# sanweiliti/RoHM

Hardware: NVIDIA H100
Metric: denoised motion clips/sec (145-frame, 1000-step PoseNet p_sample_loop) (higher is better)
Workload: dtype f32 (fp16 hi/lo error-compensated tensor-core GEMMs)

## Files before the change

### rohm_b200/csrc/attention.cu

```cuda
#include "attention.cuh"

#include <cmath>

#include "common.h"
#include "gemm.cuh"
#include "ptx.cuh"

namespace rohm {
namespace {

__device__ __forceinline__ float4 load_qkv4(const float* qkv, const float* qkv_lo, int f16, int64_t idx) {
  if (!f16) return *reinterpret_cast<const float4*>(qkv + idx);
  const uint2 h = *reinterpret_cast<const uint2*>(reinterpret_cast<const __half*>(qkv) + idx);
  const uint2 l = *reinterpret_cast<const uint2*>(reinterpret_cast<const __half*>(qkv_lo) + idx);
  const __half2 h0 = *reinterpret_cast<const __half2*>(&h.x), h1 = *reinterpret_cast<const __half2*>(&h.y);
  const __half2 l0 = *reinterpret_cast<const __half2*>(&l.x), l1 = *reinterpret_cast<const __half2*>(&l.y);
  return make_float4(__low2float(h0) + __low2float(l0), __high2float(h0) + __high2float(l0),
                     __low2float(h1) + __low2float(l1), __high2float(h1) + __high2float(l1));
}
template <int DH>
__global__ void __launch_bounds__(256) attention_kernel(const float* __restrict__ qkv, const float* __restrict__ qkv_lo,
                                                        float* __restrict__ ctx_hi, float* __restrict__ ctx_lo, int S,
                                                        int D, int H, float scale, int f16) {
  constexpr int KP = DH + 4;
// ... 359 lines not shown
  for (int i = threadIdx.x; i < 16 * NK * (DH / 8); i += blockDim.x) {
    const int s = i / (DH / 8), c = i % (DH / 8);
    const int sc = s < S ? s : S - 1;
    const uint32_t nbytes = s < S ? 16u : 0u;
    const __half* src = qkv_hi + (base + sc) * ld + h * DH + c * 8 + D;
    const uint32_t dst = ptx::smem_u32(Kh + s * P + c * 8);
    constexpr uint32_t plane = 16 * NK * P * 2;
    asm volatile("cp.async.cg.shared.global [%0], [%1], 16, %2;" ::"r"(dst), "l"(src), "r"(nbytes) : "memory");
    asm volatile("cp.async.cg.shared.global [%0], [%1], 16, %2;" ::"r"(dst + plane), "l"(src + lo_off), "r"(nbytes) : "memory");
    asm volatile("cp.async.cg.shared.global [%0], [%1], 16, %2;" ::"r"(dst + 2 * plane), "l"(src + D), "r"(nbytes) : "memory");
    asm volatile("cp.async.cg.shared.global [%0], [%1], 16, %2;" ::"r"(dst + 3 * plane), "l"(src + D + lo_off), "r"(nbytes)
                 : "memory");
  }
  asm volatile("cp.async.commit_group;" ::: "memory");

  const int r0 = warp * 16;
  const int rowA = min(r0 + g, S - 1), rowB = min(r0 + g + 8, S - 1);
  const __half* qA = qkv_hi + (base + rowA) * ld + h * DH + 2 * t;
  const int dB = (rowB - rowA) * ld;
  auto ldq = [](const __half* p) { return __ldg(reinterpret_cast<const unsigned int*>(p)); };
  uint32_t qh[4] = {ldq(qA), ldq(qA + dB), ldq(qA + 8), ldq(qA + dB + 8)};
  uint32_t ql[4] = {ldq(qA + lo_off), ldq(qA + lo_off + dB), ldq(qA + lo_off + 8), ldq(qA + lo_off + dB + 8)};
  asm volatile("cp.async.wait_group 0;" ::: "memory");
  __syncthreads();

  float acc[NT][4];
#pragma unroll
  for (int j = 0; j < NT; ++j) acc[j][0] = acc[j][1] = acc[j][2] = acc[j][3] = 0.0f;
  const int lm = lane >> 3, lr = lane & 7;
  const __half* kbase = (lm < 2 ? Kh : Kl) + lr * P + (lm & 1) * 8;
#pragma unroll 1
  for (int k = 0; k < DH / 16; ++k) {
    uint32_t ah[4], al[4];
#pragma unroll
    for (int i = 0; i < 4; ++i) ah[i] = qh[i], al[i] = ql[i];
    if (k + 1 < DH / 16) {
      const __half* q = qA + 16 * (k + 1);
      qh[0] = ldq(q), qh[1] = ldq(q + dB), qh[2] = ldq(q + 8), qh[3] = ldq(q + dB + 8);
      q += lo_off;
      ql[0] = ldq(q), ql[1] = ldq(q + dB), ql[2] = ldq(q + 8), ql[3] = ldq(q + dB + 8);
    }
    const __half* kp = kbase + 16 * k;
#pragma unroll
    for (int j0 = 0; j0 < NT; j0 += 4) {
      uint32_t bf[4][4];
#pragma unroll
      for (int u = 0; u < 4; ++u) ldmatrix_x4(bf[u], kp + (j0 + u) * 8 * P);
#pragma unroll
      for (int u = 0; u < 4; ++u) mma_f16_16x8x16(acc[j0 + u], al, bf[u][0], bf[u][1]);
#pragma unroll
      for (int u = 0; u < 4; ++u) mma_f16_16x8x16(acc[j0 + u], ah, bf[u][2], bf[u][3]);
#pragma unroll
      for (int u = 0; u < 4; ++u) mma_f16_16x8x16(acc[j0 + u], ah, bf[u][0], bf[u][1]);
    }
  }

  float mxA = -INFINITY, mxB = -INFINITY;
#pragma unroll
  for (int j = 0; j < NT; ++j) {
#pragma unroll
    for (int e = 0; e < 2; ++e) {
      const bool ok = (8 * j + 2 * t + e) < S;
      acc[j][e] = ok ? acc[j][e] * scale : -INFINITY;
      acc[j][2 + e] = ok ? acc[j][2 + e] * scale : -INFINITY;
      mxA = fmaxf(mxA, acc[j][e]);
      mxB = fmaxf(mxB, acc[j][2 + e]);
    }
  }
  mxA = fmaxf(mxA, __shfl_xor_sync(0xffffffffu, mxA, 1));
  mxA = fmaxf(mxA, __shfl_xor_sync(0xffffffffu, mxA, 2));
  mxB = fmaxf(mxB, __shfl_xor_sync(0xffffffffu, mxB, 1));
  mxB = fmaxf(mxB, __shfl_xor_sync(0xffffffffu, mxB, 2));
  float sumA = 0.0f, sumB = 0.0f;
#pragma unroll
  for (int j = 0; j < NT; ++j) {
#pragma unroll
    for (int e = 0; e < 2; ++e) {
      acc[j][e] = expf(acc[j][e] - mxA);
      acc[j][2 + e] = expf(acc[j][2 + e] - mxB);
      sumA += acc[j][e];
      sumB += acc[j][2 + e];
    }
  }
  sumA += __shfl_xor_sync(0xffffffffu, sumA, 1);
  sumA += __shfl_xor_sync(0xffffffffu, sumA, 2);
  sumB += __shfl_xor_sync(0xffffffffu, sumB, 1);
  sumB += __shfl_xor_sync(0xffffffffu, sumB, 2);
  const float invA = 1.0f / sumA, invB = 1.0f / sumB;

  uint32_t ph[NK][4], pl[NK][4];
#pragma unroll
  for (int jj = 0; jj < NK; ++jj) {
    split_f16x2(acc[2 * jj][0] * invA, acc[2 * jj][1] * invA, ph[jj][0], pl[jj][0]);
    split_f16x2(acc[2 * jj][2] * invB, acc[2 * jj][3] * invB, ph[jj][1], pl[jj][1]);
    split_f16x2(acc[2 * jj + 1][0] * invA, acc[2 * jj + 1][1] * invA, ph[jj][2], pl[jj][2]);
    split_f16x2(acc[2 * jj + 1][2] * invB, acc[2 * jj + 1][3] * invB, ph[jj][3], pl[jj][3]);
  }

  const bool okA = (r0 + g) < S, okB = (r0 + g + 8) < S;
  const int64_t oA = (base + r0 + g) * D + h * DH + 2 * t;
  const int64_t oB = oA + static_cast<int64_t>(8) * D;
  const __half* vbase = (lm < 2 ? Vh : Vl) + ((lm & 1) * 8 + lr) * P;
  constexpr int NU = 4;
#pragma unroll 1
  for (int n0 = 0; n0 < DH / 8; n0 += NU) {
    float o[NU][4];
#pragma unroll
    for (int u = 0; u < NU; ++u) o[u][0] = o[u][1] = o[u][2] = o[u][3] = 0.0f;
    const __half* vp = vbase + 8 * n0;
#pragma unroll
    for (int jj = 0; jj < NK; ++jj) {
      uint32_t bf[NU][4];
#pragma unroll
      for (int u = 0; u < NU; ++u) ldmatrix_x4_trans(bf[u], vp + 16 * jj * P + 8 * u);
#pragma unroll
      for (int u = 0; u < NU; ++u) mma_f16_16x8x16(o[u], pl[jj], bf[u][0], bf[u][1]);
#pragma unroll
      for (int u = 0; u < NU; ++u) mma_f16_16x8x16(o[u], ph[jj], bf[u][2], bf[u][3]);
#pragma unroll
      for (int u = 0; u < NU; ++u) mma_f16_16x8x16(o[u], ph[jj], bf[u][0], bf[u][1]);
    }
#pragma unroll
    for (int u = 0; u < NU; ++u) {
      const int n = n0 + u;
      uint32_t hA, lA, hB, lB;
      split_f16x2(o[u][0], o[u][1], hA, lA);
      split_f16x2(o[u][2], o[u][3], hB, lB);
      if (okA) {
        *reinterpret_cast<uint32_t*>(ctx_hi + oA + 8 * n) = hA;
        *reinterpret_cast<uint32_t*>(ctx_lo + oA + 8 * n) = lA;
      }
      if (okB) {
        *reinterpret_cast<uint32_t*>(ctx_hi + oB + 8 * n) = hB;
        *reinterpret_cast<uint32_t*>(ctx_lo + oB + 8 * n) = lB;
      }
    }
  }
}

template <int DH>
size_t attention_f16_smem_bytes(int NK) { return sizeof(__half) * 4 * 16 * NK * attn_f16_pitch<DH>(); }

struct AttnWgParams {
  CUtensorMap q_hi, q_lo;
  CUtensorMap kv_hi, kv_lo;
  __half* ctx_hi;
  __half* ctx_lo;
  int S, D, H;
  float scale;
  const int* clip_off;
  const int* clip_ids;
};
constexpr int kAwKeys = 160;
constexpr int kAwQRows = 64;
constexpr int kAwQBuf = kAwQRows * 128;
constexpr int kAwKBuf = kAwKeys * 128;
constexpr int kAwSmemBytes = 4 * kAwQBuf + 8 * kAwKBuf + 1024;

__global__ void __launch_bounds__(128, 1) attention_wgmma_kernel(const __grid_constant__ AttnWgParams p) {
  extern __shared__ uint8_t aw_smem_raw[];
  __shared__ uint64_t bar_qk, bar_v;
  const uint32_t raw = ptx::smem_u32(aw_smem_raw);
  uint8_t* const sm = aw_smem_raw + ((1024u - (raw & 1023u)) & 1023u);
  uint8_t* const Qb = sm;
  uint8_t* const Kb = sm + 4 * kAwQBuf;
  uint8_t* const Vb = Kb + 4 * kAwKBuf;
  const int qtiles = (p.S + kAwQRows - 1) / kAwQRows;
  const int qt = static_cast<int>(blockIdx.x) % qtiles;
  const int bh = static_cast<int>(blockIdx.x) / qtiles;
  const int h = bh % p.H, b = bh / p.H;
  const int q0 = qt * kAwQRows;
  int S = p.S, row0 = b * p.S;
  if (p.clip_off != nullptr) {
    const int c = p.clip_ids[b];
    row0 = p.clip_off[c];
    S = p.clip_off[c + 1] - row0;
    if (q0 >= S) return;
  }
  const int warp = threadIdx.x >> 5, lane = threadIdx.x & 31;
  if (threadIdx.x == 0) {
    ptx::prefetch_tmap(&p.q_hi);
    ptx::prefetch_tmap(&p.q_lo);
    ptx::prefetch_tmap(&p.kv_hi);
    ptx::prefetch_tmap(&p.kv_lo);
    ptx::mbar_init(&bar_qk, 1);
    ptx::mbar_init(&bar_v, 1);
    ptx::fence_barrier_init();
  }
  __syncthreads();
  ptx::pdl_launch_dependents();
  ptx::pdl_wait_prior_grid();
  if (threadIdx.x == 0) {
    ptx::mbar_expect_tx(&bar_qk, 4 * kAwQBuf + 4 * kAwKBuf);
    for (int pl = 0; pl < 2; ++pl)
      for (int c = 0; c < 2; ++c) {
        ptx::tma_load_2d(Qb + (pl * 2 + c) * kAwQBuf, pl ? &p.q_lo : &p.q_hi, &bar_qk, h * 128 + 64 * c, row0 + q0);
        ptx::tma_load_2d(Kb + (pl * 2 + c) * kAwKBuf, pl ? &p.kv_lo : &p.kv_hi, &bar_qk, p.D + h * 128 + 64 * c, row0);
      }
    ptx::mbar_expect_tx(&bar_v, 4 * kAwKBuf);
    for (int pl = 0; pl < 2; ++pl)
      for (int c = 0; c < 2; ++c)
        ptx::tma_load_2d(Vb + (pl * 2 + c) * kAwKBuf, pl ? &p.kv_lo : &p.kv_hi, &bar_v, 2 * p.D + h * 128 + 64 * c, row0);
  }

  float s[80];
#pragma unroll
  for (int i = 0; i < 80; ++i) s[i] = 0.0f;
  ptx::mbar_wait(&bar_qk, 0);
  ptx::wgmma_fence_regs(s);
  ptx::wgmma_fence();
#pragma unroll
  for (int k = 0; k < 8; ++k) {
    const int c = k >> 2;
    const uint64_t ko = static_cast<uint64_t>((k & 3) * 2);
    const uint64_t qh = ptx::make_desc_kmajor<128>(ptx::smem_u32(Qb + c * kAwQBuf)) + ko;
    const uint64_t ql = ptx::make_desc_kmajor<128>(ptx::smem_u32(Qb + (2 + c) * kAwQBuf)) + ko;
    const uint64_t kh = ptx::make_desc_kmajor<128>(ptx::smem_u32(Kb + c * kAwKBuf)) + ko;
    const uint64_t kl = ptx::make_desc_kmajor<128>(ptx::smem_u32(Kb + (2 + c) * kAwKBuf)) + ko;
    ptx::wgmma_f16(s, ql, kh);
    ptx::wgmma_f16(s, qh, kl);
    ptx::wgmma_f16(s, qh, kh);
  }
  ptx::wgmma_commit();
  ptx::wgmma_wait<0>();
  ptx::wgmma_fence_regs(s);

  const int c2 = 2 * (lane & 3);
  float m0 = -INFINITY, m1 = -INFINITY;
#pragma unroll
  for (int j = 0; j < 20; ++j) {
#pragma unroll
    for (int e = 0; e < 2; ++e) {
      const bool valid = 8 * j + c2 + e < S;
      s[4 * j + e] = valid ? s[4 * j + e] : -INFINITY;
      s[4 * j + 2 + e] = valid ? s[4 * j + 2 + e] : -INFINITY;
      m0 = fmaxf(m0, s[4 * j + e]);
      m1 = fmaxf(m1, s[4 * j + 2 + e]);
    }
  }
#pragma unroll
  for (int off = 1; off <= 2; off <<= 1) {
    m0 = fmaxf(m0, __shfl_xor_sync(0xffffffffu, m0, off));
    m1 = fmaxf(m1, __shfl_xor_sync(0xffffffffu, m1, off));
  }
  float l0 = 0.0f, l1 = 0.0f;
#pragma unroll
  for (int j = 0; j < 20; ++j) {
#pragma unroll
    for (int e = 0; e < 2; ++e) {
      const bool valid = 8 * j + c2 + e < S;
      const float p0 = valid ? expf((s[4 * j + e] - m0) * p.scale) : 0.0f;
      const float p1 = valid ? expf((s[4 * j + 2 + e] - m1) * p.scale) : 0.0f;
      s[4 * j + e] = p0, s[4 * j + 2 + e] = p1;
      l0 += p0, l1 += p1;
    }
  }
#pragma unroll
  for (int off = 1; off <= 2; off <<= 1) {
    l0 += __shfl_xor_sync(0xffffffffu, l0, off);
    l1 += __shfl_xor_sync(0xffffffffu, l1, off);
  }
  uint32_t ph[10][4], plo[10][4];
#pragma unroll
  for (int k = 0; k < 10; ++k)
#pragma unroll
    for (int i = 0; i < 4; ++i) ptx::split_f16x2(s[8 * k + 2 * i], s[8 * k + 2 * i + 1], ph[k][i], plo[k][i]);
#pragma unroll
  for (int k = 0; k < 10; ++k)
#pragma unroll
    for (int i = 0; i < 4; ++i) asm volatile("" : "+r"(ph[k][i]), "+r"(plo[k][i])::"memory");

  ptx::mbar_wait(&bar_v, 0);
  if (S < kAwKeys) {
    const int n = (kAwKeys - S) * 8;
    for (int i = threadIdx.x; i < 4 * n; i += 128) {
      const int buf = i / n, r = i - buf * n;
      *reinterpret_cast<uint4*>(Vb + buf * kAwKBuf + S * 128 + r * 16) = make_uint4(0u, 0u, 0u, 0u);
    }
    ptx::fence_proxy_async();
    __syncthreads();
  }

  float o[64];
#pragma unroll
  for (int i = 0; i < 64; ++i) o[i] = 0.0f;
  ptx::wgmma_fence_regs(o);
  ptx::wgmma_fence();
#pragma unroll
  for (int k = 0; k < 10; ++k) {
    const uint64_t vh = ptx::make_desc_mnmajor_sw128(ptx::smem_u32(Vb + k * 2048), kAwKBuf, 1024);
    const uint64_t vl = ptx::make_desc_mnmajor_sw128(ptx::smem_u32(Vb + 2 * kAwKBuf + k * 2048), kAwKBuf, 1024);
    ptx::wgmma_f16_rs_tb(o, plo[k], vh);
    ptx::wgmma_f16_rs_tb(o, ph[k], vl);
    ptx::wgmma_f16_rs_tb(o, ph[k], vh);
  }
  ptx::wgmma_commit();
  ptx::wgmma_wait<0>();
  ptx::wgmma_fence_regs(o);
#pragma unroll
  for (int k = 0; k < 10; ++k)
#pragma unroll
    for (int i = 0; i < 4; ++i) asm volatile("" : "+r"(ph[k][i]), "+r"(plo[k][i])::"memory");

  const int ra = q0 + warp * 16 + (lane >> 2), rb = ra + 8;
  const float ia = 1.0f / l0, ib = 1.0f / l1;
#pragma unroll
  for (int j = 0; j < 16; ++j) {
    const int col = h * 128 + 8 * j + c2;
    uint32_t hi, lo;
    if (ra < S) {
      ptx::split_f16x2(o[4 * j] * ia, o[4 * j + 1] * ia, hi, lo);
      const int64_t off = static_cast<int64_t>(row0 + ra) * p.D + col;
      *reinterpret_cast<uint32_t*>(p.ctx_hi + off) = hi;
      *reinterpret_cast<uint32_t*>(p.ctx_lo + off) = lo;
    }
    if (rb < S) {
      ptx::split_f16x2(o[4 * j + 2] * ib, o[4 * j + 3] * ib, hi, lo);
      const int64_t off = static_cast<int64_t>(row0 + rb) * p.D + col;
      *reinterpret_cast<uint32_t*>(p.ctx_hi + off) = hi;
      *reinterpret_cast<uint32_t*>(p.ctx_lo + off) = lo;
    }
  }
}

struct AttnStreamParams {
  CUtensorMap hi, lo;
  __half* ctx_hi;
  __half* ctx_lo;
  int S, D, H;
  float scale;
  const int* clip_off;
  const int* clip_ids;
};
constexpr int kAsBlock = 64;
constexpr int kAsBuf = kAsBlock * 128;
constexpr int kAsTile = 4 * kAsBuf;
constexpr int kAsStages = 2;
constexpr int kAsSmemBytes = (1 + 2 * kAsStages) * kAsTile + 1024;

__global__ void __launch_bounds__(128, 1) attention_wgmma_stream_kernel(const __grid_constant__ AttnStreamParams p) {
  extern __shared__ uint8_t as_smem_raw[];
  __shared__ uint64_t bar_q, bar_k[kAsStages], bar_v[kAsStages];
  const uint32_t raw = ptx::smem_u32(as_smem_raw);
  uint8_t* const sm = as_smem_raw + ((1024u - (raw & 1023u)) & 1023u);
  uint8_t* const Qb = sm;
  uint8_t* const Kb = sm + kAsTile;
  uint8_t* const Vb = Kb + kAsStages * kAsTile;
  const int qtiles = (p.S + kAsBlock - 1) / kAsBlock;
  const int qt = static_cast<int>(blockIdx.x) % qtiles;
  const int bh = static_cast<int>(blockIdx.x) / qtiles;
  const int h = bh % p.H, b = bh / p.H;
  const int q0 = qt * kAsBlock;
  int S = p.S, row0 = b * p.S;
  if (p.clip_off != nullptr) {
    const int c = p.clip_ids[b];
    row0 = p.clip_off[c];
    S = p.clip_off[c + 1] - row0;
    if (q0 >= S) return;
  }
  const int nblk = (S + kAsBlock - 1) / kAsBlock;
  const int kcol = p.D + h * 128, vcol = 2 * p.D + h * 128;
  const int warp = threadIdx.x >> 5, lane = threadIdx.x & 31;
  if (threadIdx.x == 0) {
    ptx::prefetch_tmap(&p.hi);
    ptx::prefetch_tmap(&p.lo);
    ptx::mbar_init(&bar_q, 1);
    for (int s = 0; s < kAsStages; ++s) ptx::mbar_init(&bar_k[s], 1), ptx::mbar_init(&bar_v[s], 1);
    ptx::fence_barrier_init();
  }
  __syncthreads();
  ptx::pdl_launch_dependents();
  ptx::pdl_wait_prior_grid();
  auto load_tile = [&](uint8_t* dst, uint64_t* bar, int col, int row) {
    ptx::mbar_expect_tx(bar, kAsTile);
    for (int pl = 0; pl < 2; ++pl)
      for (int c = 0; c < 2; ++c) ptx::tma_load_2d(dst + (pl * 2 + c) * kAsBuf, pl ? &p.lo : &p.hi, bar, col + 64 * c, row);
  };
  if (threadIdx.x == 0) {
    load_tile(Qb, &bar_q, h * 128, row0 + q0);
    for (int j = 0; j < kAsStages && j < nblk; ++j) {
      load_tile(Kb + j * kAsTile, &bar_k[j], kcol, row0 + j * kAsBlock);
      load_tile(Vb + j * kAsTile, &bar_v[j], vcol, row0 + j * kAsBlock);
    }
  }

  const int c2 = 2 * (lane & 3);
  float o[64];
#pragma unroll
  for (int i = 0; i < 64; ++i) o[i] = 0.0f;
  float m0 = -INFINITY, m1 = -INFINITY;
  float l0 = 0.0f, l1 = 0.0f;
  ptx::mbar_wait(&bar_q, 0);
#pragma unroll 1
  for (int j = 0; j < nblk; ++j) {
    const int st = j % kAsStages;
    const uint32_t phase = (j / kAsStages) & 1;
    uint8_t* const Ks = Kb + st * kAsTile;
    uint8_t* const Vs = Vb + st * kAsTile;
    const int kb = j * kAsBlock;

    float s[32];
#pragma unroll
    for (int i = 0; i < 32; ++i) s[i] = 0.0f;
    ptx::mbar_wait(&bar_k[st], phase);
    ptx::wgmma_fence_regs(s);
    ptx::wgmma_fence();
#pragma unroll
    for (int k = 0; k < 8; ++k) {
      const int c = k >> 2;
      const uint64_t ko = static_cast<uint64_t>((k & 3) * 2);
      const uint64_t qh = ptx::make_desc_kmajor<128>(ptx::smem_u32(Qb + c * kAsBuf)) + ko;
      const uint64_t ql = ptx::make_desc_kmajor<128>(ptx::smem_u32(Qb + (2 + c) * kAsBuf)) + ko;
      const uint64_t kh = ptx::make_desc_kmajor<128>(ptx::smem_u32(Ks + c * kAsBuf)) + ko;
      const uint64_t kl = ptx::make_desc_kmajor<128>(ptx::smem_u32(Ks + (2 + c) * kAsBuf)) + ko;
      ptx::wgmma_f16(s, ql, kh);
      ptx::wgmma_f16(s, qh, kl);
      ptx::wgmma_f16(s, qh, kh);
    }
    ptx::wgmma_commit();
    ptx::wgmma_wait<0>();
    ptx::wgmma_fence_regs(s);
    __syncthreads();
    if (threadIdx.x == 0 && j + kAsStages < nblk) load_tile(Ks, &bar_k[st], kcol, row0 + kb + kAsStages * kAsBlock);

    float n0 = m0, n1 = m1;
#pragma unroll
    for (int jj = 0; jj < 8; ++jj) {
#pragma unroll
      for (int e = 0; e < 2; ++e) {
        const bool valid = kb + 8 * jj + c2 + e < S;
        s[4 * jj + e] = valid ? s[4 * jj + e] : -INFINITY;
        s[4 * jj + 2 + e] = valid ? s[4 * jj + 2 + e] : -INFINITY;
        n0 = fmaxf(n0, s[4 * jj + e]);
        n1 = fmaxf(n1, s[4 * jj + 2 + e]);
      }
    }
#pragma unroll
    for (int off = 1; off <= 2; off <<= 1) {
      n0 = fmaxf(n0, __shfl_xor_sync(0xffffffffu, n0, off));
      n1 = fmaxf(n1, __shfl_xor_sync(0xffffffffu, n1, off));
    }
    const float a0 = expf((m0 - n0) * p.scale), a1 = expf((m1 - n1) * p.scale);
    m0 = n0, m1 = n1;
    float b0 = 0.0f, b1 = 0.0f;
#pragma unroll
    for (int jj = 0; jj < 8; ++jj) {
#pragma unroll
      for (int e = 0; e < 2; ++e) {
        const bool valid = kb + 8 * jj + c2 + e < S;
        const float p0 = valid ? expf((s[4 * jj + e] - m0) * p.scale) : 0.0f;
        const float p1 = valid ? expf((s[4 * jj + 2 + e] - m1) * p.scale) : 0.0f;
        s[4 * jj + e] = p0, s[4 * jj + 2 + e] = p1;
        b0 += p0, b1 += p1;
      }
    }
    l0 = l0 * a0 + b0, l1 = l1 * a1 + b1;
    uint32_t ph[4][4], plo[4][4];
#pragma unroll
    for (int k = 0; k < 4; ++k)
#pragma unroll
      for (int i = 0; i < 4; ++i) ptx::split_f16x2(s[8 * k + 2 * i], s[8 * k + 2 * i + 1], ph[k][i], plo[k][i]);

    ptx::mbar_wait(&bar_v[st], phase);
    if (kb + kAsBlock > S) {
      const int n = (kb + kAsBlock - S) * 8;
      for (int i = threadIdx.x; i < 4 * n; i += 128) {
        const int buf = i / n, r = i - buf * n;
        *reinterpret_cast<uint4*>(Vs + buf * kAsBuf + (S - kb) * 128 + r * 16) = make_uint4(0u, 0u, 0u, 0u);
      }
      ptx::fence_proxy_async();
      __syncthreads();
    }

    float ob[64];
#pragma unroll
    for (int i = 0; i < 64; ++i) ob[i] = 0.0f;
    ptx::wgmma_fence_regs(ob);
    ptx::wgmma_fence();
#pragma unroll
    for (int k = 0; k < 4; ++k) {
      const uint64_t vh = ptx::make_desc_mnmajor_sw128(ptx::smem_u32(Vs + k * 2048), kAsBuf, 1024);
      const uint64_t vl = ptx::make_desc_mnmajor_sw128(ptx::smem_u32(Vs + 2 * kAsBuf + k * 2048), kAsBuf, 1024);
      ptx::wgmma_f16_rs_tb(ob, plo[k], vh);
      ptx::wgmma_f16_rs_tb(ob, ph[k], vl);
      ptx::wgmma_f16_rs_tb(ob, ph[k], vh);
    }
    ptx::wgmma_commit();
    ptx::wgmma_wait<0>();
    ptx::wgmma_fence_regs(ob);
#pragma unroll
    for (int i = 0; i < 64; ++i) o[i] = fmaf(o[i], (i & 2) ? a1 : a0, ob[i]);
#pragma unroll
    for (int k = 0; k < 4; ++k)
#pragma unroll
      for (int i = 0; i < 4; ++i) asm volatile("" : "+r"(ph[k][i]), "+r"(plo[k][i])::"memory");
    __syncthreads();
    if (threadIdx.x == 0 && j + kAsStages < nblk) load_tile(Vs, &bar_v[st], vcol, row0 + kb + kAsStages * kAsBlock);
  }

#pragma unroll
  for (int off = 1; off <= 2; off <<= 1) {
    l0 += __shfl_xor_sync(0xffffffffu, l0, off);
    l1 += __shfl_xor_sync(0xffffffffu, l1, off);
  }
  const int ra = q0 + warp * 16 + (lane >> 2), rb = ra + 8;
  const float ia = 1.0f / l0, ib = 1.0f / l1;
#pragma unroll
  for (int j = 0; j < 16; ++j) {
    const int col = h * 128 + 8 * j + c2;
    uint32_t hi, lo;
    if (ra < S) {
      ptx::split_f16x2(o[4 * j] * ia, o[4 * j + 1] * ia, hi, lo);
      const int64_t off = static_cast<int64_t>(row0 + ra) * p.D + col;
      *reinterpret_cast<uint32_t*>(p.ctx_hi + off) = hi;
      *reinterpret_cast<uint32_t*>(p.ctx_lo + off) = lo;
    }
    if (rb < S) {
      ptx::split_f16x2(o[4 * j + 2] * ib, o[4 * j + 3] * ib, hi, lo);
      const int64_t off = static_cast<int64_t>(row0 + rb) * p.D + col;
      *reinterpret_cast<uint32_t*>(p.ctx_hi + off) = hi;
      *reinterpret_cast<uint32_t*>(p.ctx_lo + off) = lo;
    }
  }
}

size_t attention_mma_smem_bytes(int NT) { return sizeof(float) * 2 * 8 * NT * kAttnPitch; }

template <int DH, int NT>
cudaError_t launch_attention_mma(const AttnArgs& a, cudaStream_t st, bool pdl) {
  auto kern = attention_mma_kernel<DH, NT>;
  static bool attr_set = false;
  const size_t smem = attention_mma_smem_bytes(NT);
  if (!attr_set) {
    cudaError_t e = cudaFuncSetAttribute(kern, cudaFuncAttributeMaxDynamicSharedMemorySize, static_cast<int>(smem));
    if (e != cudaSuccess) return e;
    attr_set = true;
  }
  const int warps = (a.S + 15) / 16;
  return launch_chain(kern, dim3(a.B * a.H), dim3(32 * warps), smem, st, pdl, static_cast<const float*>(a.qkv_hi),
                      static_cast<float*>(a.ctx_hi), static_cast<float*>(a.ctx_lo), a.S, a.D, a.H, a.scale,
                      a.kind == kKindF16 ? 1 : 0);
}

template <int DH, int NK>
cudaError_t launch_attention_f16(const AttnArgs& a, cudaStream_t st, bool pdl) {
  const int warps = (a.S + 15) / 16;
  return launch_chain(attention_f16_kernel<DH, NK>, dim3(a.B * a.H), dim3(32 * warps), attention_f16_smem_bytes<DH>(NK), st,
                      pdl, static_cast<const __half*>(a.qkv_hi), static_cast<const __half*>(a.qkv_lo),
                      static_cast<__half*>(a.ctx_hi), static_cast<__half*>(a.ctx_lo), a.S, a.D, a.H, a.scale);
}

}

size_t attention_smem_bytes(int S, int DH) {
  const int Sp = (S + 31) & ~31;
  return sizeof(float) * (static_cast<size_t>(S) * (DH + 4) + static_cast<size_t>(S) * DH + 8 * DH + 8 * Sp);
}

int attention_wgmma_maps(AttnWgmmaMaps* maps, const AttnArgs& a) {
  const int D = a.D;
  int rc = make_tile_tmap_f16_sw128(&maps->q_hi, a.qkv_hi, a.rows, 3 * D, 3 * D, kAwQRows);
  if (rc == 0) rc = make_tile_tmap_f16_sw128(&maps->q_lo, a.qkv_lo, a.rows, 3 * D, 3 * D, kAwQRows);
  if (rc == 0) rc = make_tile_tmap_f16_sw128(&maps->kv_hi, a.qkv_hi, a.rows, 3 * D, 3 * D, kAwKeys);
  if (rc == 0) rc = make_tile_tmap_f16_sw128(&maps->kv_lo, a.qkv_lo, a.rows, 3 * D, 3 * D, kAwKeys);
  return rc;
}

cudaError_t attention_init_attributes(int max_tokens, int dh) {
  cudaError_t ea = cudaSuccess;
  auto set = [&](auto kern, size_t bytes) {
    if (ea == cudaSuccess) ea = cudaFuncSetAttribute(kern, cudaFuncAttributeMaxDynamicSharedMemorySize, static_cast<int>(bytes));
  };
  set(attention_mma_kernel<128, 4>, attention_mma_smem_bytes(4));
  set(attention_mma_kernel<128, 8>, attention_mma_smem_bytes(8));
  set(attention_mma_kernel<128, 12>, attention_mma_smem_bytes(12));
  set(attention_mma_kernel<128, 16>, attention_mma_smem_bytes(16));
  set(attention_mma_kernel<128, 20>, attention_mma_smem_bytes(20));
  set(attention_mma_kernel<64, 8>, attention_mma_smem_bytes(8));
  set(attention_mma_kernel<64, 20>, attention_mma_smem_bytes(20));
  set(attention_f16_kernel<128, 2>, attention_f16_smem_bytes<128>(2));
  set(attention_f16_kernel<128, 4>, attention_f16_smem_bytes<128>(4));
  set(attention_f16_kernel<128, 6>, attention_f16_smem_bytes<128>(6));
  set(attention_f16_kernel<128, 8>, attention_f16_smem_bytes<128>(8));
  set(attention_f16_kernel<128, 10>, attention_f16_smem_bytes<128>(10));
  set(attention_f16_kernel<64, 4>, attention_f16_smem_bytes<64>(4));
  set(attention_f16_kernel<64, 10>, attention_f16_smem_bytes<64>(10));
  set(attention_wgmma_kernel, kAwSmemBytes);
  set(attention_wgmma_stream_kernel, kAsSmemBytes);
  if (dh != 64 && dh != 128) return ea == cudaSuccess ? cudaErrorInvalidValue : ea;
  int simt_tokens = max_tokens < kAttnSimtMaxTokens ? max_tokens : kAttnSimtMaxTokens;
  while (simt_tokens > 1 && attention_smem_bytes(simt_tokens, dh) > kAttnSmemLimit) --simt_tokens;
  if (dh == 128) set(attention_kernel<128>, attention_smem_bytes(simt_tokens, 128));
  else set(attention_kernel<64>, attention_smem_bytes(simt_tokens, 64));
  return ea;
}

cudaError_t launch_attention(const AttnArgs& a, int which, const AttnWgmmaMaps* wg, cudaStream_t st, bool pdl) {
  const bool packed = a.clip_off != nullptr;
  if (a.B <= 0 || a.S <= 0 || a.H <= 0 || a.D % a.H != 0 || (packed ? a.S > a.rows : static_cast<int64_t>(a.B) * a.S > a.rows))
    return cudaErrorInvalidValue;
  if (packed && (a.clip_ids == nullptr || which == kAttnAuto)) return cudaErrorInvalidValue;
  const int dh = a.D / a.H;
  if (dh != 64 && dh != 128) return cudaErrorInvalidValue;
  const bool f16 = a.kind == kKindF16;
  const bool wg_ok = f16 && dh == 128 && a.S <= kAwKeys && wg != nullptr;
  const bool stream_ok = f16 && dh == 128 && wg != nullptr;
  const bool mma_ok = a.S <= kAttnWgmmaMaxTokens;
  if (which == kAttnAuto)
    which = wg_ok ? kAttnWgmma : (stream_ok && !mma_ok) ? kAttnWgmmaStream : !mma_ok ? kAttnSimt : f16 ? kAttnMmaF16 : kAttnMmaTf32;
  const int S = a.S;
  if (which == kAttnWgmmaStream) {
    if (!stream_ok) return cudaErrorInvalidValue;
    AttnStreamParams prm;
    prm.hi = wg->q_hi, prm.lo = wg->q_lo;
    prm.ctx_hi = static_cast<__half*>(a.ctx_hi), prm.ctx_lo = static_cast<__half*>(a.ctx_lo);
    prm.S = S, prm.D = a.D, prm.H = a.H, prm.scale = a.scale;
    prm.clip_off = a.clip_off, prm.clip_ids = a.clip_ids;
    const int qtiles = (S + kAsBlock - 1) / kAsBlock;
    return launch_chain(attention_wgmma_stream_kernel, dim3(a.B * a.H * qtiles), dim3(128), kAsSmemBytes, st, pdl, prm);
  }
  if (which == kAttnWgmma) {
    if (!wg_ok) return cudaErrorInvalidValue;
    AttnWgParams prm;
    prm.q_hi = wg->q_hi, prm.q_lo = wg->q_lo, prm.kv_hi = wg->kv_hi, prm.kv_lo = wg->kv_lo;
    prm.ctx_hi = static_cast<__half*>(a.ctx_hi), prm.ctx_lo = static_cast<__half*>(a.ctx_lo);
    prm.S = S, prm.D = a.D, prm.H = a.H, prm.scale = a.scale;
    prm.clip_off = a.clip_off, prm.clip_ids = a.clip_ids;
    const int qtiles = (S + kAwQRows - 1) / kAwQRows;
    return launch_chain(attention_wgmma_kernel, dim3(a.B * a.H * qtiles), dim3(128), kAwSmemBytes, st, pdl, prm);
  }
  if (packed) return cudaErrorInvalidValue;
  if (which == kAttnMmaF16) {
    if (!f16 || !mma_ok) return cudaErrorInvalidValue;
    const int nk = (S + 15) / 16;
    if (dh == 128 && nk <= 2) return launch_attention_f16<128, 2>(a, st, pdl);
    if (dh == 128 && nk <= 4) return launch_attention_f16<128, 4>(a, st, pdl);
    if (dh == 128 && nk <= 6) return launch_attention_f16<128, 6>(a, st, pdl);
    if (dh == 128 && nk <= 8) return launch_attention_f16<128, 8>(a, st, pdl);
    if (dh == 128) return launch_attention_f16<128, 10>(a, st, pdl);
    if (nk <= 4) return launch_attention_f16<64, 4>(a, st, pdl);
    return launch_attention_f16<64, 10>(a, st, pdl);
  }
  if (which == kAttnMmaTf32) {
    if (f16 || !mma_ok) return cudaErrorInvalidValue;
    const int nt = (S + 7) / 8;
    if (dh == 128 && nt <= 4) return launch_attention_mma<128, 4>(a, st, pdl);
    if (dh == 128 && nt <= 8) return launch_attention_mma<128, 8>(a, st, pdl);
    if (dh == 128 && nt <= 12) return launch_attention_mma<128, 12>(a, st, pdl);
    if (dh == 128 && nt <= 16) return launch_attention_mma<128, 16>(a, st, pdl);
    if (dh == 128) return launch_attention_mma<128, 20>(a, st, pdl);
    if (nt <= 8) return launch_attention_mma<64, 8>(a, st, pdl);
    return launch_attention_mma<64, 20>(a, st, pdl);
  }
  if (which == kAttnSimt) {
    const size_t smem = attention_smem_bytes(S, dh);
    if (S > kAttnSimtMaxTokens || smem > kAttnSmemLimit) return cudaErrorInvalidValue;
    auto kern = dh == 128 ? attention_kernel<128> : attention_kernel<64>;
    return launch_chain(kern, dim3(a.B * a.H), dim3(256), smem, st, pdl, static_cast<const float*>(a.qkv_hi),
                        static_cast<const float*>(a.qkv_lo), static_cast<float*>(a.ctx_hi), static_cast<float*>(a.ctx_lo), S,
                        a.D, a.H, a.scale, f16 ? 1 : 0);
  }
  return cudaErrorInvalidValue;
}

}
```

### rohm_b200/csrc/ptx.cuh

```cuda
#pragma once
#include <cstdint>
#include <cuda.h>
#include <cuda_fp16.h>
#include <cuda_runtime.h>

namespace rohm {
namespace ptx {

__device__ __forceinline__ uint32_t smem_u32(const void* p) {
  return static_cast<uint32_t>(__cvta_generic_to_shared(p));
}

__device__ __forceinline__ bool elect_one() {
  uint32_t pred = 0;
  asm volatile(
      "{\n\t"
      ".reg .pred P;\n\t"
      "elect.sync _|P, 0xffffffff;\n\t"
      "selp.u32 %0, 1, 0, P;\n\t"
      "}\n"
      : "=r"(pred));
  return pred != 0;
}

__device__ __forceinline__ void mbar_init(uint64_t* bar, uint32_t count) {
  asm volatile("mbarrier.init.shared::cta.b64 [%0], %1;" ::"r"(smem_u32(bar)), "r"(count));
}
__device__ __forceinline__ void fence_barrier_init() {
  asm volatile("fence.mbarrier_init.release.cluster;" ::: "memory");
}
__device__ __forceinline__ void fence_proxy_async() {
  asm volatile("fence.proxy.async.shared::cta;" ::: "memory");
}
__device__ __forceinline__ void mbar_expect_tx(uint64_t* bar, uint32_t bytes) {
  asm volatile("mbarrier.arrive.expect_tx.shared::cta.b64 _, [%0], %1;" ::"r"(smem_u32(bar)), "r"(bytes)
               : "memory");
}
__device__ __forceinline__ void mbar_arrive(uint64_t* bar) {
  asm volatile("mbarrier.arrive.shared::cta.b64 _, [%0];" ::"r"(smem_u32(bar)) : "memory");
}
__device__ __forceinline__ bool mbar_try_wait(uint64_t* bar, uint32_t parity) {
  uint32_t ok;
  asm volatile(
      "{\n\t"
      ".reg .pred P;\n\t"
      "mbarrier.try_wait.parity.shared::cta.b64 P, [%1], %2;\n\t"
      "selp.u32 %0, 1, 0, P;\n\t"
      "}\n"
      : "=r"(ok)
      : "r"(smem_u32(bar)), "r"(parity)
      : "memory");
  return ok != 0;
}
__device__ __forceinline__ void mbar_wait(uint64_t* bar, uint32_t parity) {
  while (!mbar_try_wait(bar, parity)) {
  }
}

__device__ __forceinline__ void prefetch_tmap(const CUtensorMap* m) {
  asm volatile("prefetch.tensormap [%0];" ::"l"(reinterpret_cast<uint64_t>(m)) : "memory");
}
__device__ __forceinline__ void tma_load_2d(void* smem_dst, const CUtensorMap* m, uint64_t* bar, int32_t c0,
                                            int32_t c1) {
  asm volatile(
      "cp.async.bulk.tensor.2d.shared::cluster.global.tile.mbarrier::complete_tx::bytes [%0], [%1, {%3, %4}], [%2];"
      ::"r"(smem_u32(smem_dst)),
      "l"(reinterpret_cast<uint64_t>(m)), "r"(smem_u32(bar)), "r"(c0), "r"(c1)
      : "memory");
}
__device__ __forceinline__ void tma_load_3d(void* smem_dst, const CUtensorMap* m, uint64_t* bar, int32_t c0,
                                            int32_t c1, int32_t c2) {
  asm volatile(
      "cp.async.bulk.tensor.3d.shared::cluster.global.tile.mbarrier::complete_tx::bytes [%0], [%1, {%3, %4, %5}], "
      "[%2];" ::"r"(smem_u32(smem_dst)),
      "l"(reinterpret_cast<uint64_t>(m)), "r"(smem_u32(bar)), "r"(c0), "r"(c1), "r"(c2)
      : "memory");
}

__device__ __forceinline__ void tma_store_2d(const CUtensorMap* m, const void* smem_src, int32_t c0, int32_t c1) {
  asm volatile("cp.async.bulk.tensor.2d.global.shared::cta.bulk_group [%0, {%2, %3}], [%1];" ::"l"(
                   reinterpret_cast<uint64_t>(m)),
               "r"(smem_u32(smem_src)), "r"(c0), "r"(c1)
               : "memory");
}
__device__ __forceinline__ void bulk_load_1d(void* smem_dst, const void* gsrc, uint32_t bytes, uint64_t* bar) {
  asm volatile("cp.async.bulk.shared::cluster.global.mbarrier::complete_tx::bytes [%0], [%1], %2, [%3];" ::"r"(smem_u32(smem_dst)),
               "l"(gsrc), "r"(bytes), "r"(smem_u32(bar))
               : "memory");
}
__device__ __forceinline__ void bulk_commit() { asm volatile("cp.async.bulk.commit_group;" ::: "memory"); }
__device__ __forceinline__ void bulk_wait_read_all() { asm volatile("cp.async.bulk.wait_group.read 0;" ::: "memory"); }
__device__ __forceinline__ void bulk_wait_all() { asm volatile("cp.async.bulk.wait_group 0;" ::: "memory"); }

__device__ __forceinline__ void wgmma_fence() { asm volatile("wgmma.fence.sync.aligned;" ::: "memory"); }
__device__ __forceinline__ void wgmma_commit() { asm volatile("wgmma.commit_group.sync.aligned;" ::: "memory"); }
template <int N>
__device__ __forceinline__ void wgmma_wait() {
  asm volatile("wgmma.wait_group.sync.aligned %0;" ::"n"(N) : "memory");
}
template <int R>
__device__ __forceinline__ void wgmma_fence_regs(float (&d)[R]) {
#pragma unroll
  for (int i = 0; i < R; ++i) asm volatile("" : "+f"(d[i])::"memory");
}
template <int R>
__device__ __forceinline__ void setmaxnreg_dec() {
  asm volatile("setmaxnreg.dec.sync.aligned.u32 %0;" ::"n"(R));
}
template <int R>
__device__ __forceinline__ void setmaxnreg_inc() {
  asm volatile("setmaxnreg.inc.sync.aligned.u32 %0;" ::"n"(R));
}
template <int kRowBytes>
__device__ __forceinline__ uint64_t make_desc_kmajor(uint32_t smem_addr) {
  static_assert(kRowBytes == 128 || kRowBytes == 64, "row = one swizzle span");
  uint64_t d = 0;
  d |= static_cast<uint64_t>((smem_addr & 0x3FFFFu) >> 4);
  d |= static_cast<uint64_t>(1) << 16;
  d |= static_cast<uint64_t>((8 * kRowBytes) >> 4) << 32;
  d |= static_cast<uint64_t>(kRowBytes == 128 ? 1 : 2) << 62;
  return d;
}

__device__ __forceinline__ uint64_t make_desc_mnmajor_sw128(uint32_t smem_addr, uint32_t lbo_bytes, uint32_t sbo_bytes) {
  uint64_t d = 0;
  d |= static_cast<uint64_t>((smem_addr & 0x3FFFFu) >> 4);
  d |= static_cast<uint64_t>((lbo_bytes >> 4) & 0x3FFFu) << 16;
  d |= static_cast<uint64_t>((sbo_bytes >> 4) & 0x3FFFu) << 32;
  d |= static_cast<uint64_t>(1) << 62;
  return d;
}

#define ROHM_R16_0 "%0, %1, %2, %3, %4, %5, %6, %7, %8, %9, %10, %11, %12, %13, %14, %15"
#define ROHM_R16_1 "%16, %17, %18, %19, %20, %21, %22, %23, %24, %25, %26, %27, %28, %29, %30, %31"
#define ROHM_R16_2 "%32, %33, %34, %35, %36, %37, %38, %39, %40, %41, %42, %43, %44, %45, %46, %47"
#define ROHM_R16_3 "%48, %49, %50, %51, %52, %53, %54, %55, %56, %57, %58, %59, %60, %61, %62, %63"
#define ROHM_R16_4 "%64, %65, %66, %67, %68, %69, %70, %71, %72, %73, %74, %75, %76, %77, %78, %79"
#define ROHM_F4(i) "+f"(d[i]), "+f"(d[i + 1]), "+f"(d[i + 2]), "+f"(d[i + 3])
#define ROHM_F16(i) ROHM_F4(i), ROHM_F4(i + 4), ROHM_F4(i + 8), ROHM_F4(i + 12)
#define ROHM_PRED(n) "{\n\t.reg .pred p;\n\tsetp.ne.b32 p, %" #n ", 0;\n\t"

#define ROHM_WGMMA_SS(KIND, INSTR, R, REGS, A, B, P, IMM, ...)                                                       \
  __device__ __forceinline__ void wgmma_##KIND(float (&d)[R], uint64_t desc_a, uint64_t desc_b) {                 \
    asm volatile(ROHM_PRED(P) INSTR " {" REGS "}, %" #A ", %" #B ", p" IMM ";\n\t}\n"                           \
                 : __VA_ARGS__                                                                                    \
                 : "l"(desc_a), "l"(desc_b), "r"(1));                                                             \
  }
ROHM_WGMMA_SS(f16, "wgmma.mma_async.sync.aligned.m64n32k16.f32.f16.f16", 16, ROHM_R16_0, 16, 17, 18, ", 1, 1, 0, 0",
              ROHM_F16(0))
ROHM_WGMMA_SS(f16, "wgmma.mma_async.sync.aligned.m64n64k16.f32.f16.f16", 32, ROHM_R16_0 ", " ROHM_R16_1, 32, 33, 34,
              ", 1, 1, 0, 0", ROHM_F16(0), ROHM_F16(16))
ROHM_WGMMA_SS(f16, "wgmma.mma_async.sync.aligned.m64n96k16.f32.f16.f16", 48,
              ROHM_R16_0 ", " ROHM_R16_1 ", " ROHM_R16_2, 48, 49, 50, ", 1, 1, 0, 0", ROHM_F16(0), ROHM_F16(16), ROHM_F16(32))
ROHM_WGMMA_SS(f16, "wgmma.mma_async.sync.aligned.m64n128k16.f32.f16.f16", 64,
              ROHM_R16_0 ", " ROHM_R16_1 ", " ROHM_R16_2 ", " ROHM_R16_3, 64, 65, 66, ", 1, 1, 0, 0", ROHM_F16(0),
              ROHM_F16(16), ROHM_F16(32), ROHM_F16(48))
ROHM_WGMMA_SS(f16, "wgmma.mma_async.sync.aligned.m64n160k16.f32.f16.f16", 80,
              ROHM_R16_0 ", " ROHM_R16_1 ", " ROHM_R16_2 ", " ROHM_R16_3 ", " ROHM_R16_4, 80, 81, 82, ", 1, 1, 0, 0",
              ROHM_F16(0), ROHM_F16(16), ROHM_F16(32), ROHM_F16(48), ROHM_F16(64))
ROHM_WGMMA_SS(tf32, "wgmma.mma_async.sync.aligned.m64n32k8.f32.tf32.tf32", 16, ROHM_R16_0, 16, 17, 18, ", 1, 1", ROHM_F16(0))
ROHM_WGMMA_SS(tf32, "wgmma.mma_async.sync.aligned.m64n64k8.f32.tf32.tf32", 32, ROHM_R16_0 ", " ROHM_R16_1, 32, 33, 34,
              ", 1, 1", ROHM_F16(0), ROHM_F16(16))
ROHM_WGMMA_SS(tf32, "wgmma.mma_async.sync.aligned.m64n96k8.f32.tf32.tf32", 48, ROHM_R16_0 ", " ROHM_R16_1 ", " ROHM_R16_2,
              48, 49, 50, ", 1, 1", ROHM_F16(0), ROHM_F16(16), ROHM_F16(32))
ROHM_WGMMA_SS(tf32, "wgmma.mma_async.sync.aligned.m64n128k8.f32.tf32.tf32", 64,
              ROHM_R16_0 ", " ROHM_R16_1 ", " ROHM_R16_2 ", " ROHM_R16_3, 64, 65, 66, ", 1, 1", ROHM_F16(0), ROHM_F16(16),
              ROHM_F16(32), ROHM_F16(48))

__device__ __forceinline__ void wgmma_f16_rs_tb(float (&d)[64], const uint32_t (&a)[4], uint64_t desc_b) {
  asm volatile(ROHM_PRED(69) "wgmma.mma_async.sync.aligned.m64n128k16.f32.f16.f16 {" ROHM_R16_0 ", " ROHM_R16_1 ", " ROHM_R16_2
               ", " ROHM_R16_3 "}, {%64, %65, %66, %67}, %68, p, 1, 1, 1;\n\t}\n"
               : ROHM_F16(0), ROHM_F16(16), ROHM_F16(32), ROHM_F16(48)
               : "r"(a[0]), "r"(a[1]), "r"(a[2]), "r"(a[3]), "l"(desc_b), "r"(1));
}

__device__ __forceinline__ float to_tf32(float x) {
  uint32_t r;
  asm("cvt.rna.tf32.f32 %0, %1;" : "=r"(r) : "f"(x));
  return __uint_as_float(r);
}

__device__ __forceinline__ void split_f16(float x, __half& hi, __half& lo) {
  uint16_t h;
  asm("cvt.rn.satfinite.f16.f32 %0, %1;" : "=h"(h) : "f"(x));
  hi = __ushort_as_half(h);
  lo = __float2half_rn(x - __half2float(hi));
}
__device__ __forceinline__ void split_f16x2(float x, float y, uint32_t& hi, uint32_t& lo) {
  asm("cvt.rn.satfinite.f16x2.f32 %0, %1, %2;" : "=r"(hi) : "f"(y), "f"(x));
  const float2 hf = __half22float2(*reinterpret_cast<const __half2*>(&hi));
  const float lx = x - hf.x, ly = y - hf.y;
  asm("cvt.rn.f16x2.f32 %0, %1, %2;" : "=r"(lo) : "f"(ly), "f"(lx));
}
__device__ __forceinline__ void split_f16x4(const float4& v, uint2& hi, uint2& lo) {
  split_f16x2(v.x, v.y, hi.x, lo.x);
  split_f16x2(v.z, v.w, hi.y, lo.y);
}

__device__ __forceinline__ void pdl_wait_prior_grid() { asm volatile("griddepcontrol.wait;" ::: "memory"); }
__device__ __forceinline__ void pdl_launch_dependents() { asm volatile("griddepcontrol.launch_dependents;" ::: "memory"); }

}
}
```

Before: 21.77.

## Stream K/V in 80-key blocks through one buffer to fit three CTAs per SM

```diff
diff --git a/rohm_b200/csrc/attention.cu b/rohm_b200/csrc/attention.cu
--- a/rohm_b200/csrc/attention.cu
+++ b/rohm_b200/csrc/attention.cu
@@ -535,19 +535,20 @@
   const int* clip_ids;
 };
 constexpr int kAwKeys = 160;
+constexpr int kAwBlock = 80;
 constexpr int kAwQRows = 64;
 constexpr int kAwQBuf = kAwQRows * 128;
-constexpr int kAwKBuf = kAwKeys * 128;
-constexpr int kAwSmemBytes = 4 * kAwQBuf + 8 * kAwKBuf + 1024;
-
-__global__ void __launch_bounds__(128, 1) attention_wgmma_kernel(const __grid_constant__ AttnWgParams p) {
+constexpr int kAwKBuf = kAwBlock * 128;
+constexpr int kAwSmemBytes = 4 * kAwQBuf + 4 * kAwKBuf + 1024;
+constexpr int kAwCtasPerSm = 3;
+
+__global__ void __launch_bounds__(128, kAwCtasPerSm) attention_wgmma_kernel(const __grid_constant__ AttnWgParams p) {
   extern __shared__ uint8_t aw_smem_raw[];
-  __shared__ uint64_t bar_qk, bar_v;
+  __shared__ uint64_t bar_q, bar_kv;
   const uint32_t raw = ptx::smem_u32(aw_smem_raw);
   uint8_t* const sm = aw_smem_raw + ((1024u - (raw & 1023u)) & 1023u);
   uint8_t* const Qb = sm;
-  uint8_t* const Kb = sm + 4 * kAwQBuf;
-  uint8_t* const Vb = Kb + 4 * kAwKBuf;
+  uint8_t* const KVb = sm + 4 * kAwQBuf;
   const int qtiles = (p.S + kAwQRows - 1) / kAwQRows;
   const int qt = static_cast<int>(blockIdx.x) % qtiles;
   const int bh = static_cast<int>(blockIdx.x) / qtiles;
@@ -566,47 +567,59 @@
     ptx::prefetch_tmap(&p.q_lo);
     ptx::prefetch_tmap(&p.kv_hi);
     ptx::prefetch_tmap(&p.kv_lo);
-    ptx::mbar_init(&bar_qk, 1);
-    ptx::mbar_init(&bar_v, 1);
+    ptx::mbar_init(&bar_q, 1);
+    ptx::mbar_init(&bar_kv, 1);
     ptx::fence_barrier_init();
   }
   __syncthreads();
   ptx::pdl_launch_dependents();
   ptx::pdl_wait_prior_grid();
-  if (threadIdx.x == 0) {
-    ptx::mbar_expect_tx(&bar_qk, 4 * kAwQBuf + 4 * kAwKBuf);
-    for (int pl = 0; pl < 2; ++pl)
-      for (int c = 0; c < 2; ++c) {
-        ptx::tma_load_2d(Qb + (pl * 2 + c) * kAwQBuf, pl ? &p.q_lo : &p.q_hi, &bar_qk, h * 128 + 64 * c, row0 + q0);
-        ptx::tma_load_2d(Kb + (pl * 2 + c) * kAwKBuf, pl ? &p.kv_lo : &p.kv_hi, &bar_qk, p.D + h * 128 + 64 * c, row0);
-      }
-    ptx::mbar_expect_tx(&bar_v, 4 * kAwKBuf);
+  const int kcol = p.D + h * 128, vcol = 2 * p.D + h * 128;
+  auto load_block = [&](int col, int blk) {
+    ptx::mbar_expect_tx(&bar_kv, 4 * kAwKBuf);
     for (int pl = 0; pl < 2; ++pl)
       for (int c = 0; c < 2; ++c)
-        ptx::tma_load_2d(Vb + (pl * 2 + c) * kAwKBuf, pl ? &p.kv_lo : &p.kv_hi, &bar_v, 2 * p.D + h * 128 + 64 * c, row0);
+        ptx::tma_load_2d(KVb + (pl * 2 + c) * kAwKBuf, pl ? &p.kv_lo : &p.kv_hi, &bar_kv, col + 64 * c, row0 + blk * kAwBlock);
+  };
+  if (threadIdx.x == 0) {
+    ptx::mbar_expect_tx(&bar_q, 4 * kAwQBuf);
+    for (int pl = 0; pl < 2; ++pl)
+      for (int c = 0; c < 2; ++c)
+        ptx::tma_load_2d(Qb + (pl * 2 + c) * kAwQBuf, pl ? &p.q_lo : &p.q_hi, &bar_q, h * 128 + 64 * c, row0 + q0);
+    load_block(kcol, 0);
   }
 
   float s[80];
 #pragma unroll
   for (int i = 0; i < 80; ++i) s[i] = 0.0f;
-  ptx::mbar_wait(&bar_qk, 0);
-  ptx::wgmma_fence_regs(s);
-  ptx::wgmma_fence();
-#pragma unroll
-  for (int k = 0; k < 8; ++k) {
-    const int c = k >> 2;
-    const uint64_t ko = static_cast<uint64_t>((k & 3) * 2);
-    const uint64_t qh = ptx::make_desc_kmajor<128>(ptx::smem_u32(Qb + c * kAwQBuf)) + ko;
-    const uint64_t ql = ptx::make_desc_kmajor<128>(ptx::smem_u32(Qb + (2 + c) * kAwQBuf)) + ko;
-    const uint64_t kh = ptx::make_desc_kmajor<128>(ptx::smem_u32(Kb + c * kAwKBuf)) + ko;
-    const uint64_t kl = ptx::make_desc_kmajor<128>(ptx::smem_u32(Kb + (2 + c) * kAwKBuf)) + ko;
-    ptx::wgmma_f16(s, ql, kh);
-    ptx::wgmma_f16(s, qh, kl);
-    ptx::wgmma_f16(s, qh, kh);
-  }
-  ptx::wgmma_commit();
-  ptx::wgmma_wait<0>();
-  ptx::wgmma_fence_regs(s);
+  ptx::mbar_wait(&bar_q, 0);
+#pragma unroll
+  for (int blk = 0; blk < 2; ++blk) {
+    float(&sb)[40] = *reinterpret_cast<float(*)[40]>(s + 40 * blk);
+    ptx::mbar_wait(&bar_kv, blk);
+    ptx::wgmma_fence_regs(sb);
+    ptx::wgmma_fence();
+#pragma unroll
+    for (int k = 0; k < 8; ++k) {
+      const int c = k >> 2;
+      const uint64_t ko = static_cast<uint64_t>((k & 3) * 2);
+      const uint64_t qh = ptx::make_desc_kmajor<128>(ptx::smem_u32(Qb + c * kAwQBuf)) + ko;
+      const uint64_t ql = ptx::make_desc_kmajor<128>(ptx::smem_u32(Qb + (2 + c) * kAwQBuf)) + ko;
+      const uint64_t kh = ptx::make_desc_kmajor<128>(ptx::smem_u32(KVb + c * kAwKBuf)) + ko;
+      const uint64_t kl = ptx::make_desc_kmajor<128>(ptx::smem_u32(KVb + (2 + c) * kAwKBuf)) + ko;
+      ptx::wgmma_f16(sb, ql, kh);
+      ptx::wgmma_f16(sb, qh, kl);
+      ptx::wgmma_f16(sb, qh, kh);
+    }
+    ptx::wgmma_commit();
+    ptx::wgmma_wait<0>();
+    ptx::wgmma_fence_regs(sb);
+    __syncthreads();
+    if (threadIdx.x == 0) {
+      if (blk == 0) load_block(kcol, 1);
+      else load_block(vcol, 0);
+    }
+  }
 
   const int c2 = 2 * (lane & 3);
   float m0 = -INFINITY, m1 = -INFINITY;
@@ -644,46 +657,53 @@
     l1 += __shfl_xor_sync(0xffffffffu, l1, off);
   }
   uint32_t ph[10][4], plo[10][4];
-#pragma unroll
-  for (int k = 0; k < 10; ++k)
-#pragma unroll
-    for (int i = 0; i < 4; ++i) ptx::split_f16x2(s[8 * k + 2 * i], s[8 * k + 2 * i + 1], ph[k][i], plo[k][i]);
-#pragma unroll
-  for (int k = 0; k < 10; ++k)
-#pragma unroll
-    for (int i = 0; i < 4; ++i) asm volatile("" : "+r"(ph[k][i]), "+r"(plo[k][i])::"memory");
-
-  ptx::mbar_wait(&bar_v, 0);
-  if (S < kAwKeys) {
-    const int n = (kAwKeys - S) * 8;
-    for (int i = threadIdx.x; i < 4 * n; i += 128) {
-      const int buf = i / n, r = i - buf * n;
-      *reinterpret_cast<uint4*>(Vb + buf * kAwKBuf + S * 128 + r * 16) = make_uint4(0u, 0u, 0u, 0u);
-    }
-    ptx::fence_proxy_async();
-    __syncthreads();
-  }
-
   float o[64];
 #pragma unroll
   for (int i = 0; i < 64; ++i) o[i] = 0.0f;
-  ptx::wgmma_fence_regs(o);
-  ptx::wgmma_fence();
-#pragma unroll
-  for (int k = 0; k < 10; ++k) {
-    const uint64_t vh = ptx::make_desc_mnmajor_sw128(ptx::smem_u32(Vb + k * 2048), kAwKBuf, 1024);
-    const uint64_t vl = ptx::make_desc_mnmajor_sw128(ptx::smem_u32(Vb + 2 * kAwKBuf + k * 2048), kAwKBuf, 1024);
-    ptx::wgmma_f16_rs_tb(o, plo[k], vh);
-    ptx::wgmma_f16_rs_tb(o, ph[k], vl);
-    ptx::wgmma_f16_rs_tb(o, ph[k], vh);
-  }
-  ptx::wgmma_commit();
-  ptx::wgmma_wait<0>();
-  ptx::wgmma_fence_regs(o);
-#pragma unroll
-  for (int k = 0; k < 10; ++k)
-#pragma unroll
-    for (int i = 0; i < 4; ++i) asm volatile("" : "+r"(ph[k][i]), "+r"(plo[k][i])::"memory");
+#pragma unroll
+  for (int blk = 0; blk < 2; ++blk) {
+#pragma unroll
+    for (int k = 5 * blk; k < 5 * blk + 5; ++k)
+#pragma unroll
+      for (int i = 0; i < 4; ++i) ptx::split_f16x2(s[8 * k + 2 * i], s[8 * k + 2 * i + 1], ph[k][i], plo[k][i]);
+#pragma unroll
+    for (int k = 5 * blk; k < 5 * blk + 5; ++k)
+#pragma unroll
+      for (int i = 0; i < 4; ++i) asm volatile("" : "+r"(ph[k][i]), "+r"(plo[k][i])::"memory");
+
+    ptx::mbar_wait(&bar_kv, blk);
+    const int valid = S - blk * kAwBlock;
+    if (valid < kAwBlock) {
+      const int r0 = valid > 0 ? valid : 0;
+#pragma unroll 1
+      for (int i = threadIdx.x; i < (kAwBlock - r0) * 32; i += 128)
+        *reinterpret_cast<uint4*>(KVb + (i & 3) * kAwKBuf + r0 * 128 + (i >> 2) * 16) = make_uint4(0u, 0u, 0u, 0u);
+      ptx::fence_proxy_async();
+      __syncthreads();
+    }
+    ptx::wgmma_fence_regs(o);
+    ptx::wgmma_fence();
+#pragma unroll
+    for (int kk = 0; kk < 5; ++kk) {
+      const int k = 5 * blk + kk;
+      const uint64_t vh = ptx::make_desc_mnmajor_sw128(ptx::smem_u32(KVb + kk * 2048), kAwKBuf, 1024);
+      const uint64_t vl = ptx::make_desc_mnmajor_sw128(ptx::smem_u32(KVb + 2 * kAwKBuf + kk * 2048), kAwKBuf, 1024);
+      ptx::wgmma_f16_rs_tb(o, plo[k], vh);
+      ptx::wgmma_f16_rs_tb(o, ph[k], vl);
+      ptx::wgmma_f16_rs_tb(o, ph[k], vh);
+    }
+    ptx::wgmma_commit();
+    ptx::wgmma_wait<0>();
+    ptx::wgmma_fence_regs(o);
+#pragma unroll
+    for (int kk = 0; kk < 5; ++kk)
+#pragma unroll
+      for (int i = 0; i < 4; ++i) asm volatile("" : "+r"(ph[5 * blk + kk][i]), "+r"(plo[5 * blk + kk][i])::"memory");
+    if (blk == 0) {
+      __syncthreads();
+      if (threadIdx.x == 0) load_block(vcol, 1);
+    }
+  }
 
   const int ra = q0 + warp * 16 + (lane >> 2), rb = ra + 8;
   const float ia = 1.0f / l0, ib = 1.0f / l1;
@@ -944,8 +964,8 @@
   const int D = a.D;
   int rc = make_tile_tmap_f16_sw128(&maps->q_hi, a.qkv_hi, a.rows, 3 * D, 3 * D, kAwQRows);
   if (rc == 0) rc = make_tile_tmap_f16_sw128(&maps->q_lo, a.qkv_lo, a.rows, 3 * D, 3 * D, kAwQRows);
-  if (rc == 0) rc = make_tile_tmap_f16_sw128(&maps->kv_hi, a.qkv_hi, a.rows, 3 * D, 3 * D, kAwKeys);
-  if (rc == 0) rc = make_tile_tmap_f16_sw128(&maps->kv_lo, a.qkv_lo, a.rows, 3 * D, 3 * D, kAwKeys);
+  if (rc == 0) rc = make_tile_tmap_f16_sw128(&maps->kv_hi, a.qkv_hi, a.rows, 3 * D, 3 * D, kAwBlock);
+  if (rc == 0) rc = make_tile_tmap_f16_sw128(&maps->kv_lo, a.qkv_lo, a.rows, 3 * D, 3 * D, kAwBlock);
   return rc;
 }
 
@@ -969,6 +989,11 @@
   set(attention_f16_kernel<64, 4>, attention_f16_smem_bytes<64>(4));
   set(attention_f16_kernel<64, 10>, attention_f16_smem_bytes<64>(10));
   set(attention_wgmma_kernel, kAwSmemBytes);
+  if (ea == cudaSuccess)
+    ea = cudaFuncSetAttribute(attention_wgmma_kernel, cudaFuncAttributePreferredSharedMemoryCarveout, cudaSharedmemCarveoutMaxShared);
+  int ctas = 0;
+  if (ea == cudaSuccess) ea = cudaOccupancyMaxActiveBlocksPerMultiprocessor(&ctas, attention_wgmma_kernel, 128, kAwSmemBytes);
+  if (ea == cudaSuccess && ctas < kAwCtasPerSm) ea = cudaErrorInvalidConfiguration;
   set(attention_wgmma_stream_kernel, kAsSmemBytes);
   if (dh != 64 && dh != 128) return ea == cudaSuccess ? cudaErrorInvalidValue : ea;
   int simt_tokens = max_tokens < kAttnSimtMaxTokens ? max_tokens : kAttnSimtMaxTokens;
diff --git a/rohm_b200/csrc/ptx.cuh b/rohm_b200/csrc/ptx.cuh
--- a/rohm_b200/csrc/ptx.cuh
+++ b/rohm_b200/csrc/ptx.cuh
@@ -135,7 +135,6 @@
 #define ROHM_R16_1 "%16, %17, %18, %19, %20, %21, %22, %23, %24, %25, %26, %27, %28, %29, %30, %31"
 #define ROHM_R16_2 "%32, %33, %34, %35, %36, %37, %38, %39, %40, %41, %42, %43, %44, %45, %46, %47"
 #define ROHM_R16_3 "%48, %49, %50, %51, %52, %53, %54, %55, %56, %57, %58, %59, %60, %61, %62, %63"
-#define ROHM_R16_4 "%64, %65, %66, %67, %68, %69, %70, %71, %72, %73, %74, %75, %76, %77, %78, %79"
 #define ROHM_F4(i) "+f"(d[i]), "+f"(d[i + 1]), "+f"(d[i + 2]), "+f"(d[i + 3])
 #define ROHM_F16(i) ROHM_F4(i), ROHM_F4(i + 4), ROHM_F4(i + 8), ROHM_F4(i + 12)
 #define ROHM_PRED(n) "{\n\t.reg .pred p;\n\tsetp.ne.b32 p, %" #n ", 0;\n\t"
@@ -155,9 +154,9 @@
 ROHM_WGMMA_SS(f16, "wgmma.mma_async.sync.aligned.m64n128k16.f32.f16.f16", 64,
               ROHM_R16_0 ", " ROHM_R16_1 ", " ROHM_R16_2 ", " ROHM_R16_3, 64, 65, 66, ", 1, 1, 0, 0", ROHM_F16(0),
               ROHM_F16(16), ROHM_F16(32), ROHM_F16(48))
-ROHM_WGMMA_SS(f16, "wgmma.mma_async.sync.aligned.m64n160k16.f32.f16.f16", 80,
-              ROHM_R16_0 ", " ROHM_R16_1 ", " ROHM_R16_2 ", " ROHM_R16_3 ", " ROHM_R16_4, 80, 81, 82, ", 1, 1, 0, 0",
-              ROHM_F16(0), ROHM_F16(16), ROHM_F16(32), ROHM_F16(48), ROHM_F16(64))
+ROHM_WGMMA_SS(f16, "wgmma.mma_async.sync.aligned.m64n80k16.f32.f16.f16", 40,
+              ROHM_R16_0 ", " ROHM_R16_1 ", %32, %33, %34, %35, %36, %37, %38, %39", 40, 41, 42, ", 1, 1, 0, 0", ROHM_F16(0),
+              ROHM_F16(16), ROHM_F4(32), ROHM_F4(36))
 ROHM_WGMMA_SS(tf32, "wgmma.mma_async.sync.aligned.m64n32k8.f32.tf32.tf32", 16, ROHM_R16_0, 16, 17, 18, ", 1, 1", ROHM_F16(0))
 ROHM_WGMMA_SS(tf32, "wgmma.mma_async.sync.aligned.m64n64k8.f32.tf32.tf32", 32, ROHM_R16_0 ", " ROHM_R16_1, 32, 33, 34,
               ", 1, 1", ROHM_F16(0), ROHM_F16(16))
```

After: 21.73, median of 6. About the same (-0.2%).
